# MinJunKang/DualPixelFace

Hardware: AMD Instinct MI355X
Metric: train samples/sec, StereoDPNet 1024x1536 DP pair (higher is better)
Workload: dtype f32

## Files before the change

dualpixelface_amd/csrc/conv_igemm2.hip:

```cpp
#include "conv_internal.h"
#include <type_traits>

namespace {

constexpr int MAXT = 27;
constexpr int NLD = 8;
constexpr int ZPAGE = 16;

struct G2P {
  int N, C, K, Ktot, k0;
  int ID, IH, IW, OD, OH, OW;
  int sxd, sxh, sxw;
  int e0d, e0h, e0w;
  int ext_d, ext_h;
  int pz, thp, thp_shift, odt;
  int planeStride;
  int RS, SR;
  int colshift;
  int rpc, chanStride;
  int nseg;
  int nwseg;
  int T;
  int tilesH, tilesW;
  int ntiles, cpx;
  int nchunks;
  unsigned mSR, mRPC, mEH;
  unsigned long long steps;
  int rstep;
  int accum;
  int vec;
  int single;
  double* stats;
  int statsK, statsk0;
  int tapoff[28];
  const int* wexp;
  int guard;
  int tap0, stepC, incB, incA;
};

typedef short s16x4 __attribute__((ext_vector_type(4)));
typedef __bf16 bf16x2 __attribute__((ext_vector_type(2)));
typedef float f32x2 __attribute__((ext_vector_type(2)));
typedef unsigned u32x2 __attribute__((ext_vector_type(2)));

__device__ __forceinline__ unsigned pk_bf16(float lo, float hi) {
  const f32x2 f = {lo, hi};
  return __builtin_bit_cast(unsigned, __builtin_convertvector(f, bf16x2));
}

__device__ __forceinline__ void glds16(const float* gsrc, float* ldst) {
  __builtin_amdgcn_global_load_lds((const __attribute__((address_space(1))) void*)gsrc, (__attribute__((address_space(3))) void*)ldst, 16, 0, 0);
}

template <int MT, int NT>
__device__ __forceinline__ void g2_epilogue(f32x16 (&acc)[MT][NT], const G2P& p, const float* __restrict__ bias, float* __restrict__ out, float* smem,
                                            int tile_id, int n, int qd, int q0h, int q0w, int wave, int l31, int hh, int tid) {
  constexpr int KT = 32 * MT;
  const int ow = q0w + l31;
  const long long out_plane = (long long)p.OH * p.OW;
  const long long kstride = (long long)p.OD * out_plane;
  float* op = out + ((long long)n * p.Ktot + p.k0) * kstride + ow;
  long long orow[NT];
  bool rok[NT];
#pragma unroll
  for (int t = 0; t < NT; ++t) {
    const int r = wave * NT + t, oz = qd + (r >> p.thp_shift), oy = q0h + (r & (p.thp - 1)) * p.rstep;
    rok[t] = oz < p.OD && oy < p.OH;
    orow[t] = ((long long)oz * p.OH + oy) * p.OW;
  }
  if (p.vec) {
    const int q = l31 & 3, owv = q0w + (l31 & ~3);
    const bool o1 = (q & 1) != 0, o2 = (q & 2) != 0;
    float* opv = out + ((long long)n * p.Ktot + p.k0) * kstride + owv;
#pragma unroll
    for (int m = 0; m < MT; ++m)
#pragma unroll
      for (int i = 0; i < 4; ++i) {
        const int k = m * 32 + 8 * i + 4 * hh + q;
        const float bv = (bias && k < p.K) ? bias[p.k0 + k] : 0.f;
#pragma unroll
        for (int t = 0; t < NT; ++t) {
          float r0 = acc[m][t][4 * i], r1 = acc[m][t][4 * i + 1], r2 = acc[m][t][4 * i + 2], r3 = acc[m][t][4 * i + 3];
          {
            const float x = o1 ? r0 : r1, y = o1 ? r2 : r3;
            const float xs = __builtin_bit_cast(float, __builtin_amdgcn_mov_dpp(__builtin_bit_cast(int, x), 0xB1, 0xf, 0xf, true));
            const float ys = __builtin_bit_cast(float, __builtin_amdgcn_mov_dpp(__builtin_bit_cast(int, y), 0xB1, 0xf, 0xf, true));
            if (o1) { r0 = xs; r2 = ys; } else { r1 = xs; r3 = ys; }
          }
          {
            const float x = o2 ? r0 : r2, y = o2 ? r1 : r3;
            const float xs = __builtin_bit_cast(float, __builtin_amdgcn_mov_dpp(__builtin_bit_cast(int, x), 0x4E, 0xf, 0xf, true));
            const float ys = __builtin_bit_cast(float, __builtin_amdgcn_mov_dpp(__builtin_bit_cast(int, y), 0x4E, 0xf, 0xf, true));
            if (o2) { r0 = xs; r1 = ys; } else { r2 = xs; r3 = ys; }
          }
          if (rok[t] && k < p.K && owv < p.OW) {
            f32x4* o = reinterpret_cast<f32x4*>(opv + (long long)k * kstride + orow[t]);
            f32x4 v = {r0 + bv, r1 + bv, r2 + bv, r3 + bv};
            if (p.accum) v += *o;
            *o = v;
          }
        }
      }
  } else if (ow < p.OW && !p.accum) {
#pragma unroll
    for (int m = 0; m < MT; ++m) {
#pragma unroll
      for (int j = 0; j < 16; ++j) {
        const int k = m * 32 + (j & 3) + 8 * (j >> 2) + 4 * hh;
        if (k < p.K) {
          const float bv = bias ? bias[p.k0 + k] : 0.f;
#pragma unroll
          for (int t = 0; t < NT; ++t)
            if (rok[t]) op[(long long)k * kstride + orow[t]] = acc[m][t][j] + bv;
        }
      }
    }
  } else if (ow < p.OW) {
#pragma unroll
    for (int m = 0; m < MT; ++m) {
#pragma unroll
      for (int j = 0; j < 16; ++j) {
        const int k = m * 32 + (j & 3) + 8 * (j >> 2) + 4 * hh;
        if (k < p.K) {
          const float bv = bias ? bias[p.k0 + k] : 0.f;
#pragma unroll
          for (int t = 0; t < NT; ++t)
            if (rok[t]) {
              float* o = op + (long long)k * kstride + orow[t];
              *o += acc[m][t][j] + bv;
            }
        }
      }
    }
  }
  if (p.stats) {
    double* red = reinterpret_cast<double*>(smem);
    const bool colok = ow < p.OW;
#pragma unroll
    for (int m = 0; m < MT; ++m) {
      double v1[16], v2[16];
#pragma unroll
      for (int j = 0; j < 16; ++j) {
        const int k = m * 32 + (j & 3) + 8 * (j >> 2) + 4 * hh;
        const float bv = (bias && k < p.K) ? bias[p.k0 + k] : 0.f;
        double d1 = 0.0, d2 = 0.0;
#pragma unroll
        for (int t = 0; t < NT; ++t) {
          const double v = (colok && rok[t]) ? (double)(acc[m][t][j] + bv) : 0.0;
          d1 += v;
          d2 += v * v;
        }
        v1[j] = d1;
        v2[j] = d2;
      }
#pragma unroll
      for (int half = 8; half >= 1; half >>= 1) {
        const bool upper = (l31 & (2 * half)) != 0;
#pragma unroll
        for (int i = 0; i < half; ++i) {
          const double s1 = upper ? v1[i] : v1[i + half], s2 = upper ? v2[i] : v2[i + half];
          const double k1 = upper ? v1[i + half] : v1[i], k2 = upper ? v2[i + half] : v2[i];
          v1[i] = k1 + __shfl_xor(s1, 2 * half, 64);
          v2[i] = k2 + __shfl_xor(s2, 2 * half, 64);
        }
      }
      const double r1 = v1[0] + __shfl_xor(v1[0], 1, 64), r2 = v2[0] + __shfl_xor(v2[0], 1, 64);
      if ((l31 & 1) == 0) {
        const int j = (l31 >> 1) & 15;
        double* dst = red + (((wave * 2 + hh) * MT + m) * 16 + j) * 2;
        dst[0] = r1;
        dst[1] = r2;
      }
    }
    __syncthreads();
    if (tid < KT && tid < p.K) {
      const int m = tid >> 5, kk = tid & 31;
      const int h2 = (kk >> 2) & 1, j = (kk & 3) + 4 * (kk >> 3);
      double a1 = 0.0, a2 = 0.0;
#pragma unroll
      for (int wv = 0; wv < 4; ++wv) {
        const double* src = red + (((wv * 2 + h2) * MT + m) * 16 + j) * 2;
        a1 += src[0];
        a2 += src[1];
      }
      double* row = p.stats + ((long long)tile_id * p.statsK + p.statsk0 + tid) * 2;
      row[0] = a1;
      row[1] = a2;
// ... 81 lines not shown
    }
  };

  f32x16 acc[MT][NT];
#pragma unroll
  for (int m = 0; m < MT; ++m)
#pragma unroll
    for (int t = 0; t < NT; ++t)
#pragma unroll
      for (int j = 0; j < 16; ++j) acc[m][t][j] = 0.f;

  int lanebase[NT];
#pragma unroll
  for (int t = 0; t < NT; ++t) {
    const int r = wave * NT + t, rz = r >> p.thp_shift, ry = r & (p.thp - 1);
    lanebase[t] = rz * p.sxd * p.planeStride + ry * p.sxh * p.RS + l31 * p.sxw + p.colshift + hh * (BF ? 4 : 1) * p.chanStride;
  }
  const int abase = hh * KT + l31;

  issue(0, 0);
  __syncthreads();
  const int nv = p.T;
  const int tap0 = p.tap0, stepC = p.stepC, dB = p.incB - p.stepC, dA = p.incA - p.incB, chanStride = p.chanStride;
  const unsigned long long steps = p.steps;
  const int single = p.single;
  for (int chunk = 0; chunk < p.nchunks; ++chunk) {
    const int buf = single ? 0 : chunk & 1;
    if (!single && chunk + 1 < p.nchunks) issue(chunk + 1, buf ^ 1);
    const float* s_in = smem + buf * bufFloats;
    const float* s_w = s_in + patchFloats;
    if constexpr (BF) {
      const short* s_wb = reinterpret_cast<const short*>(s_w) + (hh * KT + l31) * 4;
      s16x4 aA[MT], aB[MT];
      float bA[NT][4], bB[NT][4];
      int slotn = 0, toff = tap0, woff = 0;
      auto load_ops = [&](s16x4 (&a)[MT], float (&bb)[NT][4]) {
#pragma unroll
        for (int m = 0; m < MT; ++m) a[m] = *reinterpret_cast<const s16x4*>(s_wb + woff + m * 128);
#pragma unroll
        for (int t = 0; t < NT; ++t)
#pragma unroll
          for (int i = 0; i < 4; ++i) bb[t][i] = s_in[lanebase[t] + i * chanStride + toff];
        const unsigned code = (unsigned)(steps >> (2 * slotn)) & 3u;
        const int inc = stepC + (code > 0 ? dB : 0) + (code > 1 ? dA : 0);
        toff = code == 3 ? tap0 : toff + inc;
        woff = code == 3 ? 0 : woff + 8 * KT;
        slotn = code == 3 ? 0 : slotn + 1;
      };
      auto mfmas = [&](const s16x4 (&a)[MT], const float (&bb)[NT][4]) {
#pragma unroll
        for (int t = 0; t < NT; ++t) {
          const u32x2 u = {pk_bf16(bb[t][0], bb[t][1]), pk_bf16(bb[t][2], bb[t][3])};
          const s16x4 bv = __builtin_bit_cast(s16x4, u);
#pragma unroll
          for (int m = 0; m < MT; ++m) acc[m][t] = __builtin_amdgcn_mfma_f32_32x32x8bf16_1k(a[m], bv, acc[m][t], 0, 0, 0);
        }
      };
      auto touch = [&](const s16x4 (&a)[MT], const float (&bb)[NT][4]) {
#pragma unroll
        for (int m = 0; m < MT; ++m) asm volatile("" ::"v"(a[m]));
#pragma unroll
        for (int t = 0; t < NT; ++t)
#pragma unroll
          for (int i = 0; i < 4; ++i) asm volatile("" ::"v"(bb[t][i]));
        asm volatile("" ::: "memory");
      };
      load_ops(aA, bA);
      for (int slot = 0; slot + 1 < nv; slot += 2) {
        touch(aA, bA);
        load_ops(aB, bB);
        __builtin_amdgcn_sched_barrier(6);
        mfmas(aA, bA);
        __builtin_amdgcn_sched_barrier(0);
        touch(aB, bB);
        load_ops(aA, bA);
        __builtin_amdgcn_sched_barrier(6);
        mfmas(aB, bB);
        __builtin_amdgcn_sched_barrier(0);
      }
      if (nv & 1) mfmas(aA, bA);
    } else {
      float aA[CC / 2][MT], bA[CC / 2][NT], aB[CC / 2][MT], bB[CC / 2][NT];
      int slotn = 0, toff = tap0, woff = 0;
      auto load_ops = [&](float (&a)[CC / 2][MT], float (&bb)[CC / 2][NT]) {
        const float* wrow = s_w + abase + woff;
  #pragma unroll
        for (int cp = 0; cp < CC / 2; ++cp) {
  #pragma unroll
          for (int m = 0; m < MT; ++m) a[cp][m] = wrow[(2 * cp) * KT + m * 32];
  #pragma unroll
          for (int t = 0; t < NT; ++t) bb[cp][t] = s_in[lanebase[t] + (2 * cp) * chanStride + toff];
        }
        const unsigned code = (unsigned)(steps >> (2 * slotn)) & 3u;
        const int inc = stepC + (code > 0 ? dB : 0) + (code > 1 ? dA : 0);
        toff = code == 3 ? tap0 : toff + inc;
        woff = code == 3 ? 0 : woff + CC * KT;
        slotn = code == 3 ? 0 : slotn + 1;
      };
      auto mfmas = [&](const float (&a)[CC / 2][MT], const float (&bb)[CC / 2][NT]) {
  #pragma unroll
        for (int cp = 0; cp < CC / 2; ++cp)
  #pragma unroll
          for (int m = 0; m < MT; ++m)
  #pragma unroll
            for (int t = 0; t < NT; ++t) acc[m][t] = __builtin_amdgcn_mfma_f32_32x32x2f32(a[cp][m], bb[cp][t], acc[m][t], 0, 0, 0);
      };
      auto touch = [&](const float (&a)[CC / 2][MT], const float (&bb)[CC / 2][NT]) {
  #pragma unroll
        for (int cp = 0; cp < CC / 2; ++cp) {
  #pragma unroll
          for (int m = 0; m < MT; ++m) asm volatile("" ::"v"(a[cp][m]));
  #pragma unroll
          for (int t = 0; t < NT; ++t) asm volatile("" ::"v"(bb[cp][t]));
        }
        asm volatile("" ::: "memory");
      };
      load_ops(aA, bA);
      for (int slot = 0; slot + 1 < nv; slot += 2) {
        touch(aA, bA);
        load_ops(aB, bB);
        __builtin_amdgcn_sched_barrier(6);
        mfmas(aA, bA);
        __builtin_amdgcn_sched_barrier(0);
        touch(aB, bB);
        load_ops(aA, bA);
        __builtin_amdgcn_sched_barrier(6);
        mfmas(aB, bB);
        __builtin_amdgcn_sched_barrier(0);
      }
      if (nv & 1) mfmas(aA, bA);
    }
    __builtin_amdgcn_sched_barrier(0);
    __syncthreads();
    if (single && chunk + 1 < p.nchunks) {
      issue(chunk + 1, 0);
      __syncthreads();
    }
  }

  g2_epilogue<MT, NT>(acc, p, bias, out, smem, tile_id, n, qd, q0h, q0w, wave, l31, hh, tid);
}



typedef unsigned u32x4 __attribute__((ext_vector_type(4)));
typedef __bf16 bf16x8 __attribute__((ext_vector_type(8)));
typedef _Float16 f16x8 __attribute__((ext_vector_type(8)));

__device__ __forceinline__ void split_pair(float x, float y, unsigned& h, unsigned& m, unsigned& l) { dpf_split_pair(x, y, h, m, l); }

constexpr int X9_FIRST = DPF_X9_FIRST;
constexpr int X9_NP = 9 - X9_FIRST;

template <int CC, int NC> struct X9 {
  static constexpr int NU = CC == 4 ? 2 : 1;
  static constexpr int PB = 2 * NC * CC;
  static constexpr int TPG = 16 / CC;
  static constexpr int PD = PB / 4;
};

#ifdef DPF_STAMPS
__device__ unsigned long long g_x9_passes[4];
__device__ unsigned long long g_x9_stamps[8 * 16384];
#define X9_STAMP(slot, val) if (tid == 0 && blockIdx.x < 16384) g_x9_stamps[blockIdx.x * 8 + (slot)] = (val);
#define X9_COUNT(slot) if (tid == 0) atomicAdd(&g_x9_passes[slot], 1ull);
#else
#define X9_STAMP(slot, val)
#define X9_COUNT(slot)
#endif

template <int MT, int NT, int CC, bool SH, int NC = 3>
__global__ __launch_bounds__(256, 2) void igemm3_x9_kernel(const float* __restrict__ x, const unsigned short* __restrict__ wpk,
                                                           const float* __restrict__ bias, float* __restrict__ out, G2P p) {
  extern __shared__ __attribute__((aligned(16))) float smem[];
  static_assert(NT == 2 || NT == 4, "position rows are processed in pairs");
  constexpr int KT = 32 * MT;
  constexpr int NU = X9<CC, NC>::NU, PB = X9<CC, NC>::PB, TPG = X9<CC, NC>::TPG, PD = X9<CC, NC>::PD;
  constexpr int NPROD = NC == 3 ? X9_NP : (NC == 2 ? 3 : 1);
  constexpr int SPV = NC == 3 ? 9 : (NC == 2 ? 6 : 1);
  constexpr int NPS = NT / 2;
  constexpr int NSL = NU * 4;
  const int tid = threadIdx.x;
  const int lane = tid & 63;
  const int wave = __builtin_amdgcn_readfirstlane(tid >> 6);
  const int l31 = lane & 31;
  const int hh = lane >> 5;

  int b = (blockIdx.x & 7) * p.cpx + (blockIdx.x >> 3);
  if (b >= p.ntiles) return;
  X9_STAMP(0, __builtin_readcyclecounter()) X9_STAMP(4, __builtin_amdgcn_s_memrealtime())
  const int tile_id = b;
  const int qd = (b % p.odt) * p.pz; b /= p.odt;
  const int tw = b % p.tilesW; b /= p.tilesW;
  const int th = b % p.tilesH;
  const int n = b / p.tilesH;
  const int q0h = (th / p.rstep) * (p.thp * p.rstep) + th % p.rstep, q0w = tw * 32;
  const int i0d = qd + p.e0d, i0h = q0h + p.e0h;
  const int a0 = q0w + p.e0w - p.colshift;

  const int TG = (p.T + TPG - 1) / TPG;
  const int patchBytes = PB * p.rpc * p.RS;
  const int wBytes = TG * NC * MT * 1024;
  char* s_patch = reinterpret_cast<char*>(smem);
  char* s_w = s_patch + patchBytes;
  int* s_tab = reinterpret_cast<int*>(s_w + (SH ? 2 : 1) * wBytes);
  int* s_red = s_tab + 32;
  int Ex = DPF_H3_EMIN;
  int Erun = DPF_H3_EMIN;
  float scx = 0.f;
  unsigned tbC = 0, tbN = 0;
  unsigned kminL = 0xffffffffu;
  const long long x_chan = (long long)p.ID * p.IH * p.IW;
  const float* xn = x + (long long)n * p.C * x_chan;
  const int nunits = p.rpc * p.SR;

  if (tid < 32) s_tab[tid] = tid < 28 ? PB * p.tapoff[tid] : 0;

  int goff[NU], loff[NU];
#pragma unroll
  for (int j = 0; j < NU; ++j) {
    const unsigned f = tid + 256 * j;
    const unsigned row = (f * p.mSR) >> 20;
    const int seg = f - row * p.SR;
    const unsigned pl = (row * p.mEH) >> 20;
    const int rr = row - pl * p.ext_h;
    const int id = i0d + (int)pl, ih = i0h + rr * p.rstep, iw = a0 + 4 * seg;
    const bool ok = (int)f < nunits && id >= 0 && id < p.ID && ih >= 0 && ih < p.IH && iw >= 0 && iw < p.IW;
    goff[j] = ok ? (int)(((long long)id * p.IH + ih) * p.IW + iw) : -1;
    loff[j] = (int)f < nunits ? PB * ((int)row * p.RS + 4 * seg) : -1;
  }

  f32x4 pv[NU][CC];
  unsigned sp[NU][4][PD];
  auto prefetch = [&](int chunk) {
    const float* xc = xn + (long long)chunk * CC * x_chan;
    const int crem = p.C - chunk * CC;
#pragma unroll
    for (int j = 0; j < NU; ++j)
#pragma unroll
      for (int ch = 0; ch < CC; ++ch) {
        f32x4 v = {0.f, 0.f, 0.f, 0.f};
        if (goff[j] >= 0 && ch < crem) v = *reinterpret_cast<const f32x4*>(xc + (long long)ch * x_chan + goff[j]);
        pv[j][ch] = v;
      }
  };
  auto issue_w = [&](int chunk, int buf) {
    const char* wc = reinterpret_cast<const char*>(wpk) + (long long)chunk * wBytes;
    char* dst = s_w + buf * wBytes;
    const int nws = wBytes >> 4;
    for (int f0 = wave * 64; f0 < nws; f0 += 256) {
      const int f = f0 + lane;
      if (f < nws) glds16(reinterpret_cast<const float*>(wc + f * 16), reinterpret_cast<float*>(dst + f0 * 16));
    }
  };
  auto split_slice = [&](int sl) {
    const int j = sl >> 2, ps = sl & 3;
#pragma unroll
    for (int k = 0; k < CC / 2; ++k) {
      if constexpr (NC == 3) split_pair(pv[j][2 * k][ps], pv[j][2 * k + 1][ps], sp[j][ps][k], sp[j][ps][CC / 2 + k], sp[j][ps][CC + k]);
      else if constexpr (NC == 2) dpf_split_pair_h(pv[j][2 * k][ps] * scx, pv[j][2 * k + 1][ps] * scx, sp[j][ps][k], sp[j][ps][CC / 2 + k]);
      else sp[j][ps][k] = pk_bf16(pv[j][2 * k][ps], pv[j][2 * k + 1][ps]);
    }
  };
  auto pos_max = [&](int j, int ps) {
    float mp = __builtin_fabsf(pv[j][0][ps]);
#pragma unroll
    for (int ch = 1; ch < CC; ++ch) mp = __builtin_fmaxf(mp, __builtin_fabsf(pv[j][ch][ps]));
    return mp;
  };
  auto post_exp = [&]() {
    float pm[NU][4];
#pragma unroll
    for (int j = 0; j < NU; ++j) {
#pragma unroll
      for (int ps = 0; ps < 4; ++ps) pm[j][ps] = __builtin_fmaxf(__builtin_fabsf(pv[j][0][ps]), __builtin_fabsf(pv[j][1][ps]));
#pragma unroll
      for (int ch = 2; ch < CC; ch += 2)
#pragma unroll
        for (int ps = 0; ps < 4; ++ps) pm[j][ps] = __builtin_fmaxf(__builtin_fmaxf(pm[j][ps], __builtin_fabsf(pv[j][ch][ps])), __builtin_fabsf(pv[j][ch + 1][ps]));
    }
    float m = 0.f;
    kminL = 0xffffffffu;
#pragma unroll
    for (int j = 0; j < NU; ++j)
#pragma unroll
      for (int ps = 0; ps < 4; ps += 2) {
        m = __builtin_fmaxf(__builtin_fmaxf(m, pm[j][ps]), pm[j][ps + 1]);
        kminL = min(min(kminL, __builtin_bit_cast(unsigned, pm[j][ps]) - 1u), __builtin_bit_cast(unsigned, pm[j][ps + 1]) - 1u);
      }
    const int e = dpf_wave_max_exp(__builtin_bit_cast(unsigned, m));
    if (lane == 0) s_red[wave] = e;
  };
  auto read_exp = [&]() {
    const int4 r = *reinterpret_cast<const int4*>(s_red);
    int e = max(max(r.x, r.y), max(r.z, r.w));
    e = __builtin_amdgcn_readfirstlane(e);
    return e > 254 ? 254 : (e < DPF_H3_EMIN ? DPF_H3_EMIN : e);
  };
  auto tb_of = [&](int e) {
    return (unsigned)(e < 1 ? 1 : (e > 254 ? 254 : e)) << 23;
  };
  int Enext = Ex;
  auto next_chunk_scale = [&]() {
    const int e = read_exp();
    Erun = e > Erun ? e : Erun;
    const int lo = Erun - DPF_H3_MAXDROP;
    Enext = (e > Ex || (e < Ex - 3 && e > DPF_H3_EMIN)) ? (e > lo ? e : lo) : Ex;
    scx = dpf_h3_scale(Enext);
    tbN = p.guard ? tb_of(Enext - DPF_H3_RANGE) : 0u;
  };
  auto next_residual_scale = [&](int pass_next) {
    const int e = read_exp();
    const int lo = Erun - DPF_H3_MAXDROP;
    const int en = Ex + e - 141;
    Enext = en > lo ? en : lo;
    if (Enext > Ex) Enext = Ex;
    scx = __builtin_bit_cast(float, (unsigned)(127 + Ex - Enext) << 23);
    tbN = pass_next < DPF_H3_MAXPASS ? tb_of(Enext - DPF_H3_RANGE + 141 - Ex) : 0u;
  };
  auto lane_defers = [&](int par) {
    const bool fl = tbN != 0u && kminL < tbN - 1u;
    if (fl) s_red[8 + par] = 1;
    return __builtin_amdgcn_ballot_w64(fl) != 0ull;
  };
  auto split_masked = [&]() {
#pragma unroll
    for (int j = 0; j < NU; ++j)
#pragma unroll
      for (int ps = 0; ps < 4; ++ps) {
        const float ml = __builtin_bit_cast(unsigned, pos_max(j, ps)) >= tbN ? scx : 0.f;
#pragma unroll
        for (int k = 0; k < CC / 2; ++k) dpf_split_pair_h(pv[j][2 * k][ps] * ml, pv[j][2 * k + 1][ps] * ml, sp[j][ps][k], sp[j][ps][CC / 2 + k]);
      }
  };
  auto residual_update = [&]() {
#pragma unroll
    for (int j = 0; j < NU; ++j)
#pragma unroll
      for (int ps = 0; ps < 4; ++ps) {
        const float ml = __builtin_bit_cast(unsigned, pos_max(j, ps)) >= tbC ? 0.f : scx;
#pragma unroll
        for (int ch = 0; ch < CC; ++ch) pv[j][ch][ps] *= ml;
      }
  };
  auto store_split = [&]() {
#pragma unroll
    for (int j = 0; j < NU; ++j)
      if (loff[j] >= 0) {
        u32x4* dst = reinterpret_cast<u32x4*>(s_patch + loff[j]);
#pragma unroll
        for (int i = 0; i < PD; ++i) {
          const int e = 4 * i;
          const u32x4 v = {sp[j][e / PD][e % PD], sp[j][(e + 1) / PD][(e + 1) % PD], sp[j][(e + 2) / PD][(e + 2) % PD], sp[j][(e + 3) / PD][(e + 3) % PD]};
          dst[i] = v;
        }
      }
  };

  f32x16 acc[MT][NT];
#pragma unroll
  for (int m = 0; m < MT; ++m)
#pragma unroll
    for (int t = 0; t < NT; ++t)
#pragma unroll
      for (int j = 0; j < 16; ++j) acc[m][t][j] = 0.f;
  auto rescale_acc = [&](int de) {
#pragma unroll
    for (int m = 0; m < MT; ++m)
#pragma unroll
      for (int t = 0; t < NT; ++t)
#pragma unroll
        for (int j = 0; j < 16; ++j) acc[m][t][j] = __builtin_ldexpf(acc[m][t][j], de);
  };

  int lb[NT];
#pragma unroll
  for (int t = 0; t < NT; ++t) {
    const int r = wave * NT + t, rz = r >> p.thp_shift, ry = r & (p.thp - 1);
    lb[t] = PB * (rz * p.planeStride + ry * p.RS + l31 + p.colshift);
  }

  if constexpr (NC == 2) {
    if (tid < 2) s_red[8 + tid] = 0;
  }
  if constexpr (SH) issue_w(0, 0);
  prefetch(0);
  int par = 0;
  if constexpr (SH) {
    bool wdef = false;
    if constexpr (NC == 2) {
      post_exp();
      __syncthreads();
      next_chunk_scale();
      Ex = Enext;
      wdef = lane_defers(par);
    }
#pragma unroll
    for (int sl = 0; sl < NSL; ++sl) split_slice(sl);
    if constexpr (NC == 2) {
      if (__builtin_expect(wdef, 0)) split_masked();
    }
  }

  int pass = 0;
  for (int chunk = 0; chunk < p.nchunks;) {
    if constexpr (!SH) {
      bool wdef = false;
      if (pass == 0) issue_w(chunk, 0);
      if constexpr (NC == 2) {
        post_exp();
        __syncthreads();
        if (pass == 0) next_chunk_scale(); else next_residual_scale(pass);
        wdef = lane_defers(par);
      }
#pragma unroll
      for (int sl = 0; sl < NSL; ++sl) split_slice(sl);
      if constexpr (NC == 2) {
        if (__builtin_expect(wdef, 0)) split_masked();
      }
    }
    bool more = false;
    int dflag = 0;
    if constexpr (NC == 2) {
      if constexpr (SH) {
        if (chunk > 0 || pass > 0) dflag = s_red[8 + par];
      }
      if (tid == 0) s_red[8 + (par ^ 1)] = 0;
      if (__builtin_expect(Enext != Ex, 0)) { rescale_acc(Ex - Enext); Ex = Enext; X9_COUNT(2) }
      X9_COUNT(0)
      if (pass > 0) { X9_COUNT(1) }
      tbC = tbN;
    }
    store_split();
    __syncthreads();
    if (chunk == 0) { X9_STAMP(1, __builtin_readcyclecounter()) }
    const char* s_wc = s_w + (SH ? (chunk & 1) * wBytes : 0);
    if constexpr (NC == 2) {
      if (!SH || (chunk == 0 && pass == 0)) dflag = s_red[8 + par];
      more = pass < DPF_H3_MAXPASS && __builtin_amdgcn_readfirstlane(dflag) != 0;
      par ^= 1;
    }
    if (__builtin_expect(more, 0)) {
      residual_update();
    } else if (chunk + 1 < p.nchunks) {
      if constexpr (SH) issue_w(chunk + 1, (chunk + 1) & 1);
      prefetch(chunk + 1);
    }

    u32x4 aC[NC][MT], aN[NC][MT], bP[2][2][NC];
    int oC0, oC1 = 0, oN0 = 0, oN1 = 0;
    auto load_a = [&](int g, u32x4 (&a)[NC][MT]) {
#pragma unroll
      for (int c = 0; c < NC; ++c)
#pragma unroll
        for (int m = 0; m < MT; ++m) a[c][m] = *reinterpret_cast<const u32x4*>(s_wc + ((g * NC + c) * MT + m) * 1024 + lane * 16);
    };
    auto load_t = [&](int g, int& o0, int& o1) {
      if constexpr (CC == 4) {
        const u32x2 v = *reinterpret_cast<const u32x2*>(s_tab + 4 * g + 2 * hh);
        o0 = (int)v[0]; o1 = (int)v[1];
      } else {
        o0 = s_tab[2 * g + hh];
      }
    };
    auto load_b = [&](int t, int o0, int o1, u32x4 (&bb)[NC]) {
      if constexpr (CC == 4 && NC == 2) {
        const u32x4 q0 = *reinterpret_cast<const u32x4*>(s_patch + lb[t] + o0), q1 = *reinterpret_cast<const u32x4*>(s_patch + lb[t] + o1);
        const u32x4 vh = {q0[0], q0[1], q1[0], q1[1]}, vl = {q0[2], q0[3], q1[2], q1[3]};
        bb[0] = vh; bb[1] = vl;
      } else if constexpr (CC == 4) {
        const char* p0 = s_patch + lb[t] + o0;
        const char* p1 = s_patch + lb[t] + o1;
#pragma unroll
        for (int c = 0; c < NC; ++c) {
          const u32x2 q0 = *reinterpret_cast<const u32x2*>(p0 + 8 * c), q1 = *reinterpret_cast<const u32x2*>(p1 + 8 * c);
          const u32x4 v = {q0[0], q0[1], q1[0], q1[1]};
          bb[c] = v;
        }
      } else {
        const char* p0 = s_patch + lb[t] + o0;
#pragma unroll
        for (int c = 0; c < NC; ++c) bb[c] = *reinterpret_cast<const u32x4*>(p0 + 16 * c);
      }
    };
    auto touch_pair = [&](const u32x4 (&bb)[2][NC]) {
#pragma unroll
      for (int r = 0; r < 2; ++r)
#pragma unroll
        for (int c = 0; c < NC; ++c) asm volatile("" ::"v"(bb[r][c]));
      asm volatile("" ::: "memory");
    };
    auto touch_a = [&](const u32x4 (&a)[NC][MT]) {
#pragma unroll
      for (int c = 0; c < NC; ++c)
#pragma unroll
        for (int m = 0; m < MT; ++m) asm volatile("" ::"v"(a[c][m]));
    };
    auto mfma_pair = [&](const u32x4 (&a)[NC][MT], const u32x4 (&bb)[2][NC], int t0) {
      constexpr int oa[9] = {2, 2, 1, 2, 0, 1, 1, 0, 0};
      constexpr int ob[9] = {2, 1, 2, 0, 2, 1, 0, 1, 0};
      if constexpr (NC == 2) {
        constexpr int ha[3] = {1, 0, 0}, hb[3] = {0, 1, 0};
#pragma unroll
        for (int i = 0; i < 3; ++i)
#pragma unroll
          for (int m = 0; m < MT; ++m)
#pragma unroll
            for (int r = 0; r < 2; ++r)
              acc[m][t0 + r] = __builtin_amdgcn_mfma_f32_32x32x16_f16(__builtin_bit_cast(f16x8, a[ha[i]][m]), __builtin_bit_cast(f16x8, bb[r][hb[i]]),
                                                                       acc[m][t0 + r], 0, 0, 0);
      } else {
#pragma unroll
        for (int i = (NC == 3 ? X9_FIRST : 8); i < 9; ++i)
#pragma unroll
          for (int m = 0; m < MT; ++m)
#pragma unroll
            for (int r = 0; r < 2; ++r)
              acc[m][t0 + r] = __builtin_amdgcn_mfma_f32_32x32x16_bf16(__builtin_bit_cast(bf16x8, a[NC == 3 ? oa[i] : 0][m]),
                                                                        __builtin_bit_cast(bf16x8, bb[r][NC == 3 ? ob[i] : 0]), acc[m][t0 + r], 0, 0, 0);
      }
    };
    auto group = [&](int g, auto half_c) {
      constexpr int HALF = decltype(half_c)::value;
      const int gn = g + 1 < TG ? g + 1 : 0;
      load_t(gn, oN0, oN1);
#pragma unroll
      for (int s = 0; s < NPS; ++s) {
        touch_pair(bP[s & 1]);
        if (s == 0) touch_a(aC);
        if (s + 1 < NPS) {
          load_b(2 * s + 2, oC0, oC1, bP[(s + 1) & 1][0]);
          load_b(2 * s + 3, oC0, oC1, bP[(s + 1) & 1][1]);
        } else {
          load_a(gn, aN);
          load_b(0, oN0, oN1, bP[(s + 1) & 1][0]);
          load_b(1, oN0, oN1, bP[(s + 1) & 1][1]);
        }
        __builtin_amdgcn_sched_barrier(0);
        if constexpr (HALF >= 0) {
          constexpr int per = NSL / 2 / NPS;
#pragma unroll
          for (int q = 0; q < per; ++q) split_slice(HALF * (NSL / 2) + s * per + q);
        }
        mfma_pair(aC, bP[s & 1], 2 * s);
        if constexpr (HALF >= 0) {
          constexpr int NM = 2 * NPROD * MT;
#pragma unroll
          for (int i = 0; i < NM; ++i) {
            __builtin_amdgcn_sched_group_barrier(0x008, 1, 0);
            __builtin_amdgcn_sched_group_barrier(0x002, (NSL / 2 / NPS * CC / 2 * SPV + NM - 1) / NM + 1, 0);
          }
        }
        __builtin_amdgcn_sched_barrier(0);
      }
#pragma unroll
      for (int c = 0; c < NC; ++c)
#pragma unroll
        for (int m = 0; m < MT; ++m) aC[c][m] = aN[c][m];
      oC0 = oN0; oC1 = oN1;
      if constexpr (NPS & 1) {
#pragma unroll
        for (int r = 0; r < 2; ++r)
#pragma unroll
          for (int c = 0; c < NC; ++c) bP[0][r][c] = bP[1][r][c];
      }
    };
    load_a(0, aC);
    load_t(0, oC0, oC1);
    load_b(0, oC0, oC1, bP[0][0]);
    load_b(1, oC0, oC1, bP[0][1]);
    if constexpr (SH) {
      for (int g = 0; g + 2 < TG; ++g) group(g, std::integral_constant<int, -1>{});
      bool wdef = false;
      if constexpr (NC == 2) {
        if (more || chunk + 1 < p.nchunks) {
          post_exp();
          __syncthreads();
          if (__builtin_expect(more, 0)) next_residual_scale(pass + 1); else next_chunk_scale();
          wdef = lane_defers(par);
        }
      }
      group(TG - 2, std::integral_constant<int, 0>{});
      group(TG - 1, std::integral_constant<int, 1>{});
      if constexpr (NC == 2) {
        if (__builtin_expect(wdef, 0)) split_masked();
      }
    } else {
      for (int g = 0; g < TG; ++g) group(g, std::integral_constant<int, -1>{});
    }
    __builtin_amdgcn_sched_barrier(0);
    __syncthreads();
    if (more) ++pass;
    else { ++chunk; pass = 0; }
  }
  X9_STAMP(2, __builtin_readcyclecounter())
  if constexpr (NC == 2) { X9_COUNT(3) }
  if constexpr (NC == 2) {
#pragma unroll
    for (int m = 0; m < MT; ++m)
#pragma unroll
      for (int q4 = 0; q4 < 4; ++q4) {
        const int4 we = *reinterpret_cast<const int4*>(p.wexp + 32 * m + 8 * q4 + 4 * hh);
        const int w4[4] = {we.x, we.y, we.z, we.w};
#pragma unroll
        for (int r = 0; r < 4; ++r)
#pragma unroll
          for (int t = 0; t < NT; ++t) acc[m][t][4 * q4 + r] = __builtin_ldexpf(acc[m][t][4 * q4 + r], Ex + w4[r] - 282);
      }
  }
  g2_epilogue<MT, NT>(acc, p, bias, out, smem, tile_id, n, qd, q0h, q0w, wave, l31, hh, tid);
  X9_STAMP(3, __builtin_readcyclecounter()) X9_STAMP(5, __builtin_amdgcn_s_memrealtime()) X9_STAMP(6, (unsigned long long)__builtin_amdgcn_s_getreg((31 << 11) | 4 )) X9_STAMP(7, (unsigned long long)p.nchunks)
}

__global__ __launch_bounds__(256) void igemm3_pack_x9h_kernel(const float* __restrict__ w, unsigned short* __restrict__ wpk, int wA, int wB, int T, int TG, int MT,
                                                              int CC, int nchunks, int mode, int k0, int K, int C, int* __restrict__ wexp) {
  __shared__ int s_e[4];
  const int k = blockIdx.x, m = k >> 5, l31 = k & 31;
  const bool rowok = k < K;
  auto wat = [&](int c, int u) {
    const int a = mode == 0 ? k0 + k : c, bb = mode == 0 ? c : k0 + k;
    return w[((long long)a * wB + bb) * T + u];
  };
  float mx = 0.f;
  if (rowok)
    for (int i = threadIdx.x; i < C * T; i += 256) mx = __builtin_fmaxf(mx, __builtin_fabsf(wat(i / T, i % T)));
  const int e = dpf_wave_max_exp(__builtin_bit_cast(unsigned, mx));
  if ((threadIdx.x & 63) == 0) s_e[threadIdx.x >> 6] = e;
  __syncthreads();
  int E = max(max(s_e[0], s_e[1]), max(s_e[2], s_e[3]));
  E = E < DPF_H3_EMIN ? DPF_H3_EMIN : (E > 254 ? 254 : E);
  if (threadIdx.x == 0) wexp[k] = E;
  const float wscale = dpf_h3_scale(E);
  const int TPG = 16 / CC;
  for (int e2 = threadIdx.x; e2 < nchunks * TG * 16; e2 += 256) {
    const int i = e2 & 7, hh = (e2 >> 3) & 1, g = (e2 >> 4) % TG, chunk = (e2 >> 4) / TG;
// ... 245 lines not shown
            mfma_unit(ui, aB, bB);
            __builtin_amdgcn_sched_barrier(0);
          }
        }
      }
    }
    __syncthreads();
  }

  const int qh = q0h + wave, qw = q0w + l31;
  const long long out_plane = (long long)p.OH * p.OW;
  const long long kstride = (long long)p.OD * out_plane;
  float* on = out + ((long long)n * p.Ktot + p.k0) * kstride;
  const bool pair_ok = ((p.OW & 1) == 0) && ((reinterpret_cast<uintptr_t>(out) & 7) == 0);
  const bool quad_ok = ((p.OW & 3) == 0) && ((reinterpret_cast<uintptr_t>(out) & 15) == 0) && p.vec;
#pragma unroll
  for (int rd = 0; rd < 2; ++rd)
#pragma unroll
    for (int rh = 0; rh < 2; ++rh) {
      const int od = 2 * qd + rd, oh = 2 * qh + rh, ow = 2 * qw;
      if (od >= p.OD || oh >= p.OH || ow >= p.OW) continue;
      float* op = on + ((long long)od * p.OH + oh) * p.OW + ow;
      if (quad_ok) {
        const bool odd = (l31 & 1) != 0;
#pragma unroll
        for (int j = 0; j < 16; j += 2) {
          const float a0 = acc[rd * 4 + rh * 2][j], a1 = acc[rd * 4 + rh * 2 + 1][j];
          const float b0 = acc[rd * 4 + rh * 2][j + 1], b1 = acc[rd * 4 + rh * 2 + 1][j + 1];
          const float s0 = odd ? a0 : b0, s1 = odd ? a1 : b1;
          const float t0 = __builtin_bit_cast(float, __builtin_amdgcn_mov_dpp(__builtin_bit_cast(int, s0), 0xB1, 0xf, 0xf, true));
          const float t1 = __builtin_bit_cast(float, __builtin_amdgcn_mov_dpp(__builtin_bit_cast(int, s1), 0xB1, 0xf, 0xf, true));
          const int k = ((j + (odd ? 1 : 0)) & 3) + 8 * (j >> 2) + 4 * hh;
          if (k < p.K) {
            const float bv = bias ? bias[p.k0 + k] : 0.f;
            const f32x4 v = odd ? f32x4{t0 + bv, t1 + bv, b0 + bv, b1 + bv} : f32x4{a0 + bv, a1 + bv, t0 + bv, t1 + bv};
            *reinterpret_cast<f32x4*>(on + ((long long)od * p.OH + oh) * p.OW + (ow & ~3) + (long long)k * kstride) = v;
          }
        }
        continue;
      }
#pragma unroll
      for (int j = 0; j < 16; ++j) {
        const int k = (j & 3) + 8 * (j >> 2) + 4 * hh;
        if (k < p.K) {
          const float bv = bias ? bias[p.k0 + k] : 0.f;
          const float v0 = acc[rd * 4 + rh * 2][j] + bv, v1 = acc[rd * 4 + rh * 2 + 1][j] + bv;
          float* o = op + (long long)k * kstride;
          if (pair_ok) {
            *reinterpret_cast<float2*>(o) = make_float2(v0, v1);
          } else {
            o[0] = v0;
            if (ow + 1 < p.OW) o[1] = v1;
          }
        }
      }
    }
}

__global__ void igemm2_pack_kernel(const float* __restrict__ w, float* __restrict__ wpk, int wA, int wB, int T, int KT, int CC, int nchunks,
                                   int mode, int k0, int K, int C) {
  const long long total = (long long)nchunks * T * CC * KT + ZPAGE;
  for (long long i = (long long)blockIdx.x * blockDim.x + threadIdx.x; i < total; i += (long long)gridDim.x * blockDim.x) {
    float v = 0.f;
    if (i >= ZPAGE) {
      const long long e = i - ZPAGE;
      const int k = (int)(e % KT);
      const int cc = (int)((e / KT) % CC);
      const int t = (int)((e / ((long long)KT * CC)) % T);
      const int chunk = (int)(e / ((long long)KT * CC * T));
      const int c = chunk * CC + cc;
      if (k < K && c < C) {
        const int a = mode == 0 ? k0 + k : c;
        const int bb = mode == 0 ? c : k0 + k;
        v = w[((long long)a * wB + bb) * T + t];
      }
    }
    wpk[i] = v;
  }
}

__global__ void igemm2_pack_bf16_kernel(const float* __restrict__ w, unsigned short* __restrict__ wpk, int wA, int wB, int T, int KT, int nchunks,
                                        int mode, int k0, int K, int C) {
  const long long total = (long long)nchunks * T * 8 * KT + 2 * ZPAGE;
  for (long long i = (long long)blockIdx.x * blockDim.x + threadIdx.x; i < total; i += (long long)gridDim.x * blockDim.x) {
    float v = 0.f;
    if (i >= 2 * ZPAGE) {
      const long long e = i - 2 * ZPAGE;
      const int ii = (int)(e & 3);
      const int k = (int)((e >> 2) % KT);
      const int half = (int)((e / (4LL * KT)) & 1);
      const int t = (int)((e / (8LL * KT)) % T);
      const int chunk = (int)(e / (8LL * KT * T));
      const int c = chunk * 8 + half * 4 + ii;
      if (k < K && c < C) {
        const int a = mode == 0 ? k0 + k : c;
        const int bb = mode == 0 ? c : k0 + k;
        v = w[((long long)a * wB + bb) * T + t];
      }
    }
    wpk[i] = (unsigned short)(pk_bf16(v, 0.f) & 0xffffu);
  }
}

unsigned magic20(int d) { return (unsigned)(((1u << 20) + d - 1) / d); }

template <typename W, typename P>
struct TileLaunch {
  const float* x; const W* wpk; const float* bias; float* out; const P& p; size_t lds; long long blocks; hipStream_t st;
};

template <int MT, int NT, int CC, bool BF = false>
int launch_g2(const TileLaunch<float, G2P>& a) {
  return conv_launch<igemm2_kernel<MT, NT, CC, BF>>(dim3((unsigned)a.blocks), dim3(256), a.lds, a.st, a.x, a.wpk, a.bias, a.out, a.p);
}
template <int MT, int NT, int CC>
int launch_x9(bool sh, int NC, const TileLaunch<unsigned short, G2P>& a) {
  const dim3 grid((unsigned)a.blocks), block(256);
  switch (2 * NC + (sh ? 1 : 0)) {
    case 7: return conv_launch<igemm3_x9_kernel<MT, NT, CC, true, 3>>(grid, block, a.lds, a.st, a.x, a.wpk, a.bias, a.out, a.p);
    case 6: return conv_launch<igemm3_x9_kernel<MT, NT, CC, false, 3>>(grid, block, a.lds, a.st, a.x, a.wpk, a.bias, a.out, a.p);
    case 5: return conv_launch<igemm3_x9_kernel<MT, NT, CC, true, 2>>(grid, block, a.lds, a.st, a.x, a.wpk, a.bias, a.out, a.p);
    case 4: return conv_launch<igemm3_x9_kernel<MT, NT, CC, false, 2>>(grid, block, a.lds, a.st, a.x, a.wpk, a.bias, a.out, a.p);
    case 3: return conv_launch<igemm3_x9_kernel<MT, NT, CC, true, 1>>(grid, block, a.lds, a.st, a.x, a.wpk, a.bias, a.out, a.p);
    default: return conv_launch<igemm3_x9_kernel<MT, NT, CC, false, 1>>(grid, block, a.lds, a.st, a.x, a.wpk, a.bias, a.out, a.p);
  }
}
template <int CC, bool BF = false>
int launch_t2(const TileLaunch<float, T2P>& a) {
  return conv_launch<igemm2_tr2_kernel<CC, BF>>(dim3((unsigned)a.blocks), dim3(256), a.lds, a.st, a.x, a.wpk, a.bias, a.out, a.p);
}

int launch_x9(int MT, int NT, int CC9, bool sh, int NC, const TileLaunch<unsigned short, G2P>& a) {
  if (CC9 == 4) {
    if (MT == 1) return NT == 4 ? launch_x9<1, 4, 4>(sh, NC, a) : launch_x9<1, 2, 4>(sh, NC, a);
    return launch_x9<2, 2, 4>(sh, NC, a);
  }
  if (MT == 1) return NT == 4 ? launch_x9<1, 4, 8>(sh, NC, a) : launch_x9<1, 2, 8>(sh, NC, a);
  return launch_x9<2, 2, 8>(sh, NC, a);
}

int x9_try(const float* x, const float* w, const float* bias, float* out, float* ws, const DpfConvDesc& d, const G2P& p, int k_off, int kn, int NT,
           DpfConvStats* stats, hipStream_t st, int NC, int mt_fit = 0) {
  const ConvEnv& env = conv_env();
  constexpr int x9_min_c = 8;
  const int T = d.kd * d.kh * d.kw, MT = (kn + 31) / 32, TH = 4 * NT;
  if (!env.igemm3 || (NC >= 2 && !dpf_conv_f32_x9()) || MT > 2 || NT * MT > 4 || d.C < x9_min_c) return DPF_ERR_UNSUPPORTED;
  G2P q = p;
  q.K = kn; q.k0 = d.k0 + k_off;
  q.rstep = (env.igemm3_rstep && d.kd == 1 && d.kh > 1 && d.dh > 1) ? d.dh : 1;
  const int dhl = d.dh / q.rstep;
  int CC9 = ((T + 1) / 2) * 2 < ((T + 3) / 4) * 4 ? 8 : 4;
  if (env.igemm3_cc == 4 || env.igemm3_cc == 8) CC9 = env.igemm3_cc;
  const int NU9 = CC9 == 4 ? 2 : 1, PB9 = 2 * NC * CC9;
  auto set_pz = [&](int pz) {
    q.pz = pz; q.thp = TH / pz; q.thp_shift = 0;
    while ((1 << q.thp_shift) < q.thp) ++q.thp_shift;
    q.odt = dpf_div_up(d.OD, pz);
    q.ext_d = (pz - 1) + (d.kd - 1) * d.dd + 1;
    q.ext_h = (q.thp - 1) + (d.kh - 1) * dhl + 1;
    q.planeStride = q.ext_h * q.RS; q.SR = q.RS / 4; q.rpc = q.ext_d * q.ext_h;
    return q.rpc * q.SR;
  };
  const int TG = (T + 16 / CC9 - 1) / (16 / CC9);
  int best = 0, best_units = 1 << 30, sh = 0;
  for (int shc : {1, 0}) {
    if (best || (env.igemm3_sh >= 0 && shc != env.igemm3_sh)) continue;
    for (int pz : {1, 2, 4}) {
      if (!(pz == 1 || (d.kd > 1 && pz <= TH / 2 && pz <= d.OD))) continue;
      const int units = set_pz(pz);
      const size_t l9 = (size_t)PB9 * q.rpc * q.RS + (size_t)(shc ? 2 : 1) * TG * NC * (mt_fit > MT ? mt_fit : MT) * 1024 + 256;
      if (units <= NU9 * 256 && 2 * l9 <= 160 * 1024 && units < best_units) { best = pz; best_units = units; sh = shc; }
    }
  }
  if (!best || TG < 2) return DPF_ERR_UNSUPPORTED;
  set_pz(best);
  const size_t lds9 = (size_t)PB9 * q.rpc * q.RS + (size_t)(sh ? 2 : 1) * TG * NC * MT * 1024 + 256;
  if ((long long)NU9 * 256 * (q.SR > q.ext_h ? q.SR : q.ext_h) >= (1LL << 20)) return DPF_ERR_UNSUPPORTED;
  const int sgn = d.transposed ? -1 : 1;
  const int t0 = d.transposed ? ((d.kd - 1) * d.dd * q.ext_h + (d.kh - 1) * dhl) * q.RS + (d.kw - 1) * d.dw : 0;
  for (int u = 0; u < 28; ++u) {
    const int c = u % d.kw, b2 = (u / d.kw) % d.kh, a = u / (d.kw * d.kh);
    q.tapoff[u] = u < T ? t0 + sgn * ((a * d.dd * q.ext_h + b2 * dhl) * q.RS + c * d.dw) : 0;
  }
  q.nchunks = (d.C + CC9 - 1) / CC9;
  q.tilesH = dpf_div_up(d.OH, q.thp * q.rstep) * q.rstep;
  q.tilesW = dpf_div_up(d.OW, 32);
  q.mSR = magic20(q.SR); q.mEH = magic20(q.ext_h);
  const long long nt9 = (long long)d.N * q.odt * q.tilesH * q.tilesW;
  if (nt9 <= 0 || nt9 > 0x3fffffffLL) return DPF_ERR_INVALID_ARG;
  q.ntiles = (int)nt9;
  q.cpx = (int)((nt9 + 7) / 8);
  q.stats = nullptr;
  if (stats) {
    if (nt9 * d.K * 2 > stats->capacity_doubles) return DPF_ERR_UNSUPPORTED;
    if (k_off > 0 && stats->parts != (int)nt9) return DPF_ERR_LAUNCH;
    q.stats = stats->slab; q.statsK = d.K; q.statsk0 = k_off;
  }
  unsigned short* wp = reinterpret_cast<unsigned short*>(ws);
  const long long total = (long long)q.nchunks * TG * MT * 512;
  int* wexp = reinterpret_cast<int*>(wp + ((total * NC + 7) & ~7LL));
  q.wexp = wexp;
  q.guard = dpf_h3_range_guard();
  if (NC == 2)
    hipLaunchKernelGGL(igemm3_pack_x9h_kernel, dim3(32 * MT), dim3(256), 0, st, w, wp, d.wA, d.wB, T, TG, MT, CC9, q.nchunks, d.mode, q.k0, kn, d.C, wexp);
  else
    hipLaunchKernelGGL(igemm3_pack_x9_kernel, dim3(dpf_ew_grid(total)), dim3(256), 0, st, w, wp, d.wA, d.wB, T, TG, MT, CC9, NC, q.nchunks, d.mode, q.k0, kn,
                       d.C);
  if (dpf_check_launch() != DPF_OK) return DPF_ERR_LAUNCH;
  if (stats) stats->parts = (int)nt9;
  return launch_x9(MT, NT, CC9, sh != 0, NC, {x, wp, bias, out, q, lds9, 8LL * q.cpx, st});
}

int igemm2_tr2(const float* x, const float* w, const float* bias, float* out, float* ws, const DpfConvDesc& d, hipStream_t st) {
  if (!conv_env().igemm2_tr2) return DPF_ERR_UNSUPPORTED;
  if (d.kd != 3 || d.kh != 3 || d.kw != 3 || d.sd != 2 || d.sh != 2 || d.sw != 2 || d.pd != 1 || d.ph != 1 || d.pw != 1 || d.dd != 1 ||
      d.dh != 1 || d.dw != 1)
    return DPF_ERR_UNSUPPORTED;
  if (d.OD > 2 * d.ID || d.OH > 2 * d.IH || d.OW > 2 * d.IW) return DPF_ERR_UNSUPPORTED;
  const long long x_chan = (long long)d.ID * d.IH * d.IW;
  if (9 * x_chan >= (1LL << 30)) return DPF_ERR_UNSUPPORTED;
  const bool bf = dpf_conv_operand_bf16() != 0;
  const int CC = 8;
  T2P p{};
  p.N = d.N; p.C = d.C; p.Ktot = d.Ktot;
  p.ID = d.ID; p.IH = d.IH; p.IW = d.IW; p.OD = d.OD; p.OH = d.OH; p.OW = d.OW;
  p.RS = 36; p.SR = 9; p.rpc = 2 * 5; p.chanStride = p.rpc * p.RS;
  p.nseg = CC * p.rpc * p.SR;
  p.nwseg = bf ? 27 * 32 : 27 * CC * 32 / 4;
  p.nchunks = (d.C + CC - 1) / CC;
  p.QD = dpf_div_up(d.OD, 2);
  p.tilesH = dpf_div_up(dpf_div_up(d.OH, 2), 4);
  p.tilesW = dpf_div_up(dpf_div_up(d.OW, 2), 32);
  const long long ntiles = (long long)d.N * p.QD * p.tilesH * p.tilesW;
  if (ntiles <= 0 || ntiles > 0x3fffffffLL) return DPF_ERR_INVALID_ARG;
  p.ntiles = (int)ntiles;
  p.cpx = (int)((ntiles + 7) / 8);
  p.mSR = magic20(p.SR); p.mRPC = magic20(p.rpc); p.mEH = magic20(5);
  p.vec = conv_env().g2_vec_store;
  const size_t lds = 2 * (size_t)(CC * p.chanStride + 4 * p.nwseg) * sizeof(float);
  for (int k0 = 0; k0 < d.K; k0 += 32) {
    const int Kc = d.K - k0 < 32 ? d.K - k0 : 32;
    p.K = Kc; p.k0 = d.k0 + k0;
    const long long total = (long long)p.nchunks * 27 * CC * 32 + ZPAGE;
    if (bf)
      hipLaunchKernelGGL(igemm2_pack_bf16_kernel, dim3(dpf_ew_grid(total)), dim3(256), 0, st, w, reinterpret_cast<unsigned short*>(ws), d.wA, d.wB, 27,
                         32, p.nchunks, d.mode, p.k0, Kc, d.C);
    else
      hipLaunchKernelGGL(igemm2_pack_kernel, dim3(dpf_ew_grid(total)), dim3(256), 0, st, w, ws, d.wA, d.wB, 27, 32, CC, p.nchunks, d.mode, p.k0, Kc, d.C);
    if (dpf_check_launch() != DPF_OK) return DPF_ERR_LAUNCH;
    const TileLaunch<float, T2P> a{x, ws, bias, out, p, lds, 8LL * p.cpx, st};
    int rc;
    if (bf) rc = launch_t2<8, true>(a);
    else switch (CC) { case 2: rc = launch_t2<2>(a); break; case 4: rc = launch_t2<4>(a); break; default: rc = launch_t2<8>(a); break; }
    if (rc != DPF_OK) return rc;
  }
  return DPF_OK;
}

struct G2Plan {
  G2P p;
  int T, MT, KT;
  int NT;
  int single;
  bool bf_mode;
  bool bf;
  int CC;
};

bool g2_eligible(const float* x, const float* ws, const DpfConvDesc& d, const DpfConvStats* stats) {
  const int T = d.kd * d.kh * d.kw;
  if (!conv_env().igemm2 || T > MAXT || d.K > 128) return false;
  if ((d.IW & 3) || (reinterpret_cast<uintptr_t>(x) & 15) || (reinterpret_cast<uintptr_t>(ws) & 15)) return false;
  if (9LL * d.ID * d.IH * d.IW >= (1LL << 30)) return false;
  if (T == 1 && !conv_env().igemm2_1x1) return false;
  if (stats && (d.transposed || d.Ktot != d.K)) return false;
  return !(d.accumulate && d.transposed && (d.sd != 1 || d.sh != 1 || d.sw != 1));
}

void g2_bf16_tile(const DpfConvDesc& d, G2Plan& g) {
  const int MT = g.MT;
  g.NT = MT == 1 ? 4 : 2;
  g.bf_mode = g.bf = dpf_conv_operand_bf16() != 0 && g.T > 1;
  if (!g.bf) return;
  auto patch_for = [&](int nt) {
    const int sxh = d.transposed ? 1 : d.sh, sxw = d.transposed ? 1 : d.sw;
    const int e0w = d.transposed ? d.pw - (d.kw - 1) * d.dw : -d.pw;
    const int ext_d = (d.kd - 1) * d.dd + 1, ext_h = (4 * nt - 1) * sxh + (d.kh - 1) * d.dh + 1, ext_w = 31 * sxw + (d.kw - 1) * d.dw + 1;
    const int rs = ((((e0w % 4) + 4) % 4 + ext_w + 3) / 4) * 4;
    return (long long)8 * ext_d * ext_h * rs * 4;
  };
  const long long wbytes = (long long)g.T * g.KT * 16;
  auto occ_regs = [&](int nt) {
    const int est = MT * nt * 16 + 2 * (2 * MT + 4 * nt) + 2 * NLD + 44;
    return est <= 128 ? 4 : (est <= 168 ? 3 : 2);
  };
  int best = -1;
  for (int nt : {4, 2}) {
    if ((nt == 4 && MT > 2) || patch_for(nt) > 2LL * NLD * 256 * 16) continue;
    for (int single = 0; single < 2; ++single) {
      const long long lds_c = (single ? 1 : 2) * (patch_for(nt) + wbytes);
      if (lds_c > 160 * 1024) continue;
      int resid = (int)(160 * 1024 / lds_c);
      if (resid > occ_regs(nt)) resid = occ_regs(nt);
      if (resid > 3) resid = 3;
      const int score = resid * 4 + (single ? 0 : 2) + (nt == 4 ? 1 : 0);
      if (score > best) { best = score; g.NT = nt; g.single = single; }
    }
  }
  g.bf = best >= 0;
}

void g2_geometry(const DpfConvDesc& d, const float* out, G2Plan& g) {
  G2P& p = g.p;
  const int TH = 4 * g.NT;
  p.N = d.N; p.C = d.C; p.K = d.K; p.Ktot = d.Ktot; p.k0 = d.k0;
  p.ID = d.ID; p.IH = d.IH; p.IW = d.IW; p.OD = d.OD; p.OH = d.OH; p.OW = d.OW;
  p.T = g.T;
  p.accum = d.accumulate;
  p.rstep = 1;
  p.vec = conv_env().g2_vec_store && (d.OW & 3) == 0 && (reinterpret_cast<uintptr_t>(out) & 15) == 0;
  if (!d.transposed) {
    p.sxd = d.sd; p.sxh = d.sh; p.sxw = d.sw;
    p.e0d = -d.pd; p.e0h = -d.ph; p.e0w = -d.pw;
  } else {
    p.sxd = p.sxh = p.sxw = 1;
    p.e0d = d.pd - (d.kd - 1) * d.dd; p.e0h = d.ph - (d.kh - 1) * d.dh; p.e0w = d.pw - (d.kw - 1) * d.dw;
  }
  const int ext_w = 31 * p.sxw + (d.kw - 1) * d.dw + 1;
  p.colshift = ((p.e0w % 4) + 4) % 4;
// ... 173 lines not shown
```

Before: 27.55.

## Remap x9 patch staging rows and pad LDS rows to cut bank conflicts

Changes how threads in the x9 implicit-GEMM kernel map to patch rows when staging input into LDS. Groups of 8 consecutive threads now cover 8 different rows at the same segment rather than consecutive segments of one row. Each LDS row gets 1-2 padding positions, and for CC=8/NC=2 the hi and lo split planes are stored as separate 16-byte-strided planes. The goal is fewer LDS bank conflicts on both the split-pattern stores and the MFMA B-operand loads. In exchange, global loads across a wavefront become less coalesced and LDS use grows slightly.

```diff
diff --git a/dualpixelface_amd/csrc/conv_igemm2.hip b/dualpixelface_amd/csrc/conv_igemm2.hip
--- a/dualpixelface_amd/csrc/conv_igemm2.hip
+++ b/dualpixelface_amd/csrc/conv_igemm2.hip
@@ -33,6 +33,7 @@
   double* stats;
   int statsK, statsk0;
   int tapoff[28];
+  int rows8;
   const int* wexp;
   int guard;
   int tap0, stepC, incB, incA;
@@ -420,12 +421,19 @@
 constexpr int X9_FIRST = DPF_X9_FIRST;
 constexpr int X9_NP = 9 - X9_FIRST;
 
+#ifndef DPF_X9_ROWMAP
+#define DPF_X9_ROWMAP 1
+#endif
+constexpr bool X9_ROWMAP = DPF_X9_ROWMAP != 0;
 template <int CC, int NC> struct X9 {
   static constexpr int NU = CC == 4 ? 2 : 1;
   static constexpr int PB = 2 * NC * CC;
   static constexpr int TPG = 16 / CC;
   static constexpr int PD = PB / 4;
+  static constexpr bool PL = X9_ROWMAP && CC == 8 && NC == 2;
+  static constexpr int PA = PL ? 16 : PB;
 };
+constexpr int x9_row_pad(int CC, int NC) { return !X9_ROWMAP ? 0 : ((2 * NC * CC) % 16 == 0 ? 1 : 2); }
 
 #ifdef DPF_STAMPS
 __device__ unsigned long long g_x9_passes[4];
@@ -443,7 +451,8 @@
   extern __shared__ __attribute__((aligned(16))) float smem[];
   static_assert(NT == 2 || NT == 4, "position rows are processed in pairs");
   constexpr int KT = 32 * MT;
-  constexpr int NU = X9<CC, NC>::NU, PB = X9<CC, NC>::PB, TPG = X9<CC, NC>::TPG, PD = X9<CC, NC>::PD;
+  constexpr int NU = X9<CC, NC>::NU, PB = X9<CC, NC>::PB, TPG = X9<CC, NC>::TPG, PD = X9<CC, NC>::PD, PA = X9<CC, NC>::PA;
+  constexpr bool PL = X9<CC, NC>::PL;
   constexpr int NPROD = NC == 3 ? X9_NP : (NC == 2 ? 3 : 1);
   constexpr int SPV = NC == 3 ? 9 : (NC == 2 ? 6 : 1);
   constexpr int NPS = NT / 2;
@@ -468,6 +477,7 @@
 
   const int TG = (p.T + TPG - 1) / TPG;
   const int patchBytes = PB * p.rpc * p.RS;
+  const int planeBytes = 16 * p.rpc * p.RS;
   const int wBytes = TG * NC * MT * 1024;
   char* s_patch = reinterpret_cast<char*>(smem);
   char* s_w = s_patch + patchBytes;
@@ -480,22 +490,32 @@
   unsigned kminL = 0xffffffffu;
   const long long x_chan = (long long)p.ID * p.IH * p.IW;
   const float* xn = x + (long long)n * p.C * x_chan;
-  const int nunits = p.rpc * p.SR;
-
-  if (tid < 32) s_tab[tid] = tid < 28 ? PB * p.tapoff[tid] : 0;
+
+  if (tid < 32) s_tab[tid] = tid < 28 ? PA * p.tapoff[tid] : 0;
 
   int goff[NU], loff[NU];
 #pragma unroll
   for (int j = 0; j < NU; ++j) {
     const unsigned f = tid + 256 * j;
-    const unsigned row = (f * p.mSR) >> 20;
-    const int seg = f - row * p.SR;
+    const unsigned n8 = p.rows8 * p.SR;
+    unsigned row;
+    int seg;
+    if (f < n8) {
+      const unsigned grp = f >> 3, rb = (grp * p.mSR) >> 20;
+      seg = grp - rb * p.SR;
+      row = 8 * rb + (f & 7);
+    } else {
+      const unsigned r2 = ((f - n8) * p.mSR) >> 20;
+      seg = f - n8 - r2 * p.SR;
+      row = p.rows8 + r2;
+    }
     const unsigned pl = (row * p.mEH) >> 20;
     const int rr = row - pl * p.ext_h;
     const int id = i0d + (int)pl, ih = i0h + rr * p.rstep, iw = a0 + 4 * seg;
-    const bool ok = (int)f < nunits && id >= 0 && id < p.ID && ih >= 0 && ih < p.IH && iw >= 0 && iw < p.IW;
+    const bool unit = (int)row < p.rpc;
+    const bool ok = unit && id >= 0 && id < p.ID && ih >= 0 && ih < p.IH && iw >= 0 && iw < p.IW;
     goff[j] = ok ? (int)(((long long)id * p.IH + ih) * p.IW + iw) : -1;
-    loff[j] = (int)f < nunits ? PB * ((int)row * p.RS + 4 * seg) : -1;
+    loff[j] = unit ? PA * ((int)row * p.RS + 4 * seg) : -1;
   }
 
   f32x4 pv[NU][CC];
@@ -616,11 +636,21 @@
     for (int j = 0; j < NU; ++j)
       if (loff[j] >= 0) {
         u32x4* dst = reinterpret_cast<u32x4*>(s_patch + loff[j]);
-#pragma unroll
-        for (int i = 0; i < PD; ++i) {
-          const int e = 4 * i;
-          const u32x4 v = {sp[j][e / PD][e % PD], sp[j][(e + 1) / PD][(e + 1) % PD], sp[j][(e + 2) / PD][(e + 2) % PD], sp[j][(e + 3) / PD][(e + 3) % PD]};
-          dst[i] = v;
+        if constexpr (PL) {
+          u32x4* dlo = reinterpret_cast<u32x4*>(s_patch + loff[j] + planeBytes);
+#pragma unroll
+          for (int ps = 0; ps < 4; ++ps) {
+            const u32x4 vh = {sp[j][ps][0], sp[j][ps][1], sp[j][ps][2], sp[j][ps][3]}, vl = {sp[j][ps][4], sp[j][ps][5], sp[j][ps][6], sp[j][ps][7]};
+            dst[ps] = vh;
+            dlo[ps] = vl;
+          }
+        } else {
+#pragma unroll
+          for (int i = 0; i < PD; ++i) {
+            const int e = 4 * i;
+            const u32x4 v = {sp[j][e / PD][e % PD], sp[j][(e + 1) / PD][(e + 1) % PD], sp[j][(e + 2) / PD][(e + 2) % PD], sp[j][(e + 3) / PD][(e + 3) % PD]};
+            dst[i] = v;
+          }
         }
       }
   };
@@ -645,7 +675,7 @@
 #pragma unroll
   for (int t = 0; t < NT; ++t) {
     const int r = wave * NT + t, rz = r >> p.thp_shift, ry = r & (p.thp - 1);
-    lb[t] = PB * (rz * p.planeStride + ry * p.RS + l31 + p.colshift);
+    lb[t] = PA * (rz * p.planeStride + ry * p.RS + l31 + p.colshift);
   }
 
   if constexpr (NC == 2) {
@@ -748,7 +778,7 @@
       } else {
         const char* p0 = s_patch + lb[t] + o0;
 #pragma unroll
-        for (int c = 0; c < NC; ++c) bb[c] = *reinterpret_cast<const u32x4*>(p0 + 16 * c);
+        for (int c = 0; c < NC; ++c) bb[c] = *reinterpret_cast<const u32x4*>(p0 + (PL ? planeBytes : 16) * c);
       }
     };
     auto touch_pair = [&](const u32x4 (&bb)[2][NC]) {
@@ -1300,13 +1330,15 @@
   int CC9 = ((T + 1) / 2) * 2 < ((T + 3) / 4) * 4 ? 8 : 4;
   if (env.igemm3_cc == 4 || env.igemm3_cc == 8) CC9 = env.igemm3_cc;
   const int NU9 = CC9 == 4 ? 2 : 1, PB9 = 2 * NC * CC9;
+  q.SR = p.RS / 4;
+  q.RS = 4 * q.SR + x9_row_pad(CC9, NC);
   auto set_pz = [&](int pz) {
     q.pz = pz; q.thp = TH / pz; q.thp_shift = 0;
     while ((1 << q.thp_shift) < q.thp) ++q.thp_shift;
     q.odt = dpf_div_up(d.OD, pz);
     q.ext_d = (pz - 1) + (d.kd - 1) * d.dd + 1;
     q.ext_h = (q.thp - 1) + (d.kh - 1) * dhl + 1;
-    q.planeStride = q.ext_h * q.RS; q.SR = q.RS / 4; q.rpc = q.ext_d * q.ext_h;
+    q.planeStride = q.ext_h * q.RS; q.rpc = q.ext_d * q.ext_h;
     return q.rpc * q.SR;
   };
   const int TG = (T + 16 / CC9 - 1) / (16 / CC9);
@@ -1323,6 +1355,7 @@
   if (!best || TG < 2) return DPF_ERR_UNSUPPORTED;
   set_pz(best);
   const size_t lds9 = (size_t)PB9 * q.rpc * q.RS + (size_t)(sh ? 2 : 1) * TG * NC * MT * 1024 + 256;
+  q.rows8 = X9_ROWMAP ? q.rpc / 8 * 8 : 0;
   if ((long long)NU9 * 256 * (q.SR > q.ext_h ? q.SR : q.ext_h) >= (1LL << 20)) return DPF_ERR_UNSUPPORTED;
   const int sgn = d.transposed ? -1 : 1;
   const int t0 = d.transposed ? ((d.kd - 1) * d.dd * q.ext_h + (d.kh - 1) * dhl) * q.RS + (d.kw - 1) * d.dw : 0;
```

Measured after the change: 27.48. No clear change (-0.3%).
